# MingyuKim87/Safe_Denoiser

Measured on AMD Instinct MI355X. Metric: images/sec (512x512, 50 steps, SD-v1.4 + repellency), higher is better.
Workload: dtype bf16; 1 GPU; README-default end to end (safree = svf = lra = true, safree_neg_prompt_config.json:26-28): token ids -> CLIP -> SAFREE projection -> DDPM 50 steps x UNet on 3 guidance branches with per-prompt text switching + safe_denoiser.yaml repellency (kernel_fast, M=515, sigma 3.15, scale .33, margin 1.6, window 780<=t<=1000) -> VAE decode -> uint8 512x512 images; SD-v1.4 UNet / CLIP / VAE with random weigh; guidance_branches=3, text_encoder_precision=bf16x3, prompts_per_batch=64, latent_repeat=3, renoise_draws_rank0=3520, parallelism=prompt-shard x1

## Files before the change

safe_denoiser_amd/csrc/sdn_attn.hip:

```cpp
#include <stdlib.h>

#include <type_traits>

#include "sdn_common.h"
#include "sdn_ops.h"

namespace sdn_attn_detail {

typedef __attribute__((ext_vector_type(4))) short s16x4;
typedef __attribute__((ext_vector_type(16))) float f32x16;
typedef __attribute__((ext_vector_type(4))) unsigned int u32x4;

#if defined(__HIP_DEVICE_COMPILE__)
__device__ __forceinline__ __amdgpu_buffer_rsrc_t make_rsrc(const void* p, unsigned bytes) {
  return __builtin_amdgcn_make_buffer_rsrc(const_cast<void*>(p), 0, (int)bytes, 0x00020000);
}
typedef __attribute__((address_space(3))) void* lds_ptr_t;
#endif

#ifdef SDN_ATTN_STAMPS
#define SDN_ATS_DECL unsigned long long ats_prev = 0, ats_sum[7] = {0, 0, 0, 0, 0, 0, 0};
#define SDN_ATS_T0 unsigned long long ats_t0; asm volatile("s_memtime %0\n\ts_waitcnt lgkmcnt(0)" : "=s"(ats_t0)::"memory");
#define SDN_ATS_MARK(I)                                                                         \
  {                                                                                             \
    unsigned long long t_;                                                                      \
    asm volatile("s_memtime %0\n\ts_waitcnt lgkmcnt(0)" : "=s"(t_)::"memory");                  \
    if ((I) >= 0) ats_sum[(I) < 0 ? 0 : (I)] += t_ - ats_prev;                                  \
    ats_prev = t_;                                                                              \
  }
#define SDN_ATS_FLUSH                                                                           \
  if (g_attn_stamps && lane == 0)                                                               \
    for (int i_ = 0; i_ < 7; ++i_) g_attn_stamps[((long)blockIdx.x * 4 + wid) * 7 + i_] = ats_sum[i_];
__device__ unsigned long long* g_attn_stamps = nullptr;
#define SDN_ATS_PRO ats_sum[5] = ats_prev - ats_t0;
#else
#define SDN_ATS_DECL
#define SDN_ATS_T0
#define SDN_ATS_PRO
#define SDN_ATS_MARK(I)
#define SDN_ATS_FLUSH
#endif

constexpr int THREADS = 256;
[[maybe_unused]] constexpr int KV = 64;
constexpr int QB = 128;

struct AttnArgs {
  const unsigned short* q; const unsigned short* k; const unsigned short* v; unsigned short* out;
  int nq, nk, ldq, ldk, ldv, ldo;
  float c;
  int heads, nqb, npairs;
  const unsigned short* q2; const unsigned short* k2; const unsigned short* v2; unsigned short* out2;
  int n1, ldq2, ldk2, ldv2, ldo2;
  int head_inner;
  int causal; const int* kmask;
  int nomax;
  const float* bias;
};

template <bool SEG>
__device__ __forceinline__ const unsigned short* row_ptr(const unsigned short* p1, const unsigned short* p2, int ld1,
                                                          int ld2, int n1, int n, int b, int row) {
  if (SEG && row >= n1) return p2 + ((long)b * (n - n1) + (row - n1)) * ld2;
  return p1 + ((long)b * (SEG ? n1 : n) + row) * ld1;
}

template <typename T, int HD, bool SEG, bool MASK = false, bool DMA = !SEG, int QS = 1, bool BIAS = false>
__global__ void __launch_bounds__(THREADS)
k_attn(const AttnArgs a) {
#if defined(__HIP_DEVICE_COMPILE__)
  SDN_ATS_T0
  constexpr int KQ = (HD + 15) / 16;
  constexpr int NDB = (HD + 31) / 32;
  constexpr bool ONES = (HD % 32) != 0;
  static_assert(!BIAS || (MASK && DMA && QS == 1), "the biased form extends the masked single-buffer instance");
  constexpr bool OFFSET_FREE = T::kDtype == 0 && !BIAS;
  constexpr bool CENTRED = T::kDtype == 1 && !SEG && !MASK && DMA && (KQ * 16 > HD);
  constexpr bool CENTRED_SUB = T::kDtype == 1 && !MASK && !CENTRED;
  constexpr bool QSCALED = OFFSET_FREE || CENTRED || CENTRED_SUB;
  static_assert(!CENTRED || ((HD % 32) != 0 && HD - 16 * (KQ - 1) == 8), "centred form: row sums by the ones column, column HD = element 0 of the h = 1 lanes");
  constexpr int CH = HD / 8;
#ifndef SDN_ATTN_VCH40
#define SDN_ATTN_VCH40 5
#endif
  constexpr int KCH = HD == 40 ? 5 : CH + 1;
  constexpr int VCH = HD == 40 ? SDN_ATTN_VCH40 : (HD == 160 ? 20 : 12);
  constexpr int KSTR = DMA ? KCH * 16 : KQ * 32 + 16;
  constexpr int VSTR_PAD = (NDB * 16) % 64 == 16 || (NDB * 16) % 64 == 48 ? NDB * 64 : NDB * 64 + 64;
  constexpr int VSTR = DMA ? VCH * 16 : VSTR_PAD;
  constexpr int STAGE = KV * KSTR + KV * VSTR;
  constexpr int ZOFF = 2 * STAGE;
  constexpr int NLOAD = (2 * KV * CH + THREADS - 1) / THREADS;
  constexpr int BOFF = ZOFF + 64;
  __shared__ __attribute__((aligned(1024))) unsigned char smem[BIAS ? BOFF + 4096 : 2 * STAGE + 48];

  constexpr bool kLateDma = HD == 40;
#ifdef SDN_ATTN_NO_ASM_TR
  constexpr bool kAsmTrOn = false;
#else
  constexpr bool kAsmTrOn = true;
#endif
  const int tid = threadIdx.x, lane = tid & 63;
  const int wid = __builtin_amdgcn_readfirstlane(tid >> 6);
  const int r = lane & 31, h = lane >> 5;
  int pair, qblk;
  {
    const int nqb = a.nqb, npairs = a.npairs, id = blockIdx.x;
    if (a.head_inner) {
      const int x = id & 7, j = id >> 3;
      const int hh = j % a.heads, rest = j / a.heads;
      qblk = rest % nqb;
      pair = ((rest / nqb) * 8 + x) * a.heads + hh;
    } else if ((npairs & 7) == 0) {
      const int x = id & 7, j = id >> 3;
      pair = (j / nqb) * 8 + x; qblk = j - (j / nqb) * nqb;
    } else {
      pair = id / nqb; qblk = id - pair * nqb;
    }
  }
  const int head = pair % a.heads, b = pair / a.heads;
  const int q0 = qblk * (QB * QS) + wid * (32 * QS);
  bool qvalid[QS];
#pragma unroll
  for (int qs = 0; qs < QS; ++qs) qvalid[qs] = q0 + 32 * qs + r < a.nq;

  if (tid == 8) *reinterpret_cast<unsigned*>(smem + ZOFF + 32) = 0u;
  if constexpr (DMA) {
    if (tid < 8) *reinterpret_cast<unsigned*>(smem + ZOFF + tid * 4) = tid == 0 ? (T::pack2(1.0f, 0.0f) & 0xffffu) : 0u;
  } else {
    const unsigned one16 = T::pack2(1.0f, 0.0f) & 0xffffu;
    for (int e = tid; e < 2 * KV; e += THREADS) {
      unsigned char* sK = smem + (e / KV) * STAGE + (e % KV) * KSTR;
      unsigned char* sV = smem + (e / KV) * STAGE + KV * KSTR + (e % KV) * VSTR;
      for (int c = CH * 16; c < KQ * 32; c += 4) *reinterpret_cast<unsigned*>(sK + c) = 0u;
      for (int c = CH * 16; c < NDB * 64; c += 4) *reinterpret_cast<unsigned*>(sV + c) = (ONES && c == CH * 16) ? one16 : 0u;
    }
  }

  if constexpr (BIAS) {
    const int L = 2 * a.nk - 1;
    for (int e = tid; e < L; e += THREADS)
      reinterpret_cast<float*>(smem + BOFF)[e] = a.bias[(long)head * L + e] * 1.4426950408889634f;
  }

  typename T::v8 qf[QS][KQ];
#pragma unroll
  for (int qs = 0; qs < QS; ++qs)
#pragma unroll
  for (int s = 0; s < KQ; ++s) {
    const int dc = 16 * s + 8 * h;
    u32x4 v = (u32x4){0u, 0u, 0u, 0u};
    if (qvalid[qs] && dc < HD)
      v = *reinterpret_cast<const u32x4*>(row_ptr<SEG>(a.q, a.q2, a.ldq, a.ldq2, a.n1, a.nq, b, q0 + 32 * qs + r) + head * HD + dc);
    if (QSCALED) {
      v.x = T::pack2(T::to_f(v.x & 0xffff) * a.c, T::to_f(v.x >> 16) * a.c);
      v.y = T::pack2(T::to_f(v.y & 0xffff) * a.c, T::to_f(v.y >> 16) * a.c);
      v.z = T::pack2(T::to_f(v.z & 0xffff) * a.c, T::to_f(v.z >> 16) * a.c);
      v.w = T::pack2(T::to_f(v.w & 0xffff) * a.c, T::to_f(v.w >> 16) * a.c);
    }
    qf[qs][s] = *reinterpret_cast<typename T::v8*>(&v);
  }

  u32x4 stg[NLOAD];
  int ld_row[NLOAD], ld_dst[NLOAD];
  const unsigned short* ld_src[NLOAD];
  long ld_stride[NLOAD];
#pragma unroll
  for (int i = 0; i < NLOAD; ++i) {
    int e = tid + i * THREADS;
    const bool live = e < 2 * KV * CH;
    if (!live) e = 2 * KV * CH - 1;
    const int isv = e >= KV * CH;
    const int e2 = isv ? e - KV * CH : e;
    const int row = e2 / CH, ch = e2 - row * CH;
    ld_row[i] = row;
    ld_dst[i] = live ? (isv ? KV * KSTR + row * VSTR : row * KSTR) + ch * 16 : -1;
    ld_src[i] = (isv ? a.v + (long)b * a.nk * a.ldv : a.k + (long)b * a.nk * a.ldk) + head * HD + ch * 8;
    ld_stride[i] = isv ? a.ldv : a.ldk;
    if (SEG) { ld_stride[i] = isv; ld_src[i] = nullptr; ld_row[i] |= ch << 16; }
  }
  auto g_load = [&](int t) {
    const int k0 = t * KV;
#pragma unroll
    for (int i = 0; i < NLOAD; ++i) {
      if (SEG) {
        const int krow = min(k0 + (ld_row[i] & 0xffff), a.nk - 1), ch = ld_row[i] >> 16;
        const unsigned short* rp = ld_stride[i] ? row_ptr<true>(a.v, a.v2, a.ldv, a.ldv2, a.n1, a.nk, b, krow)
                                                : row_ptr<true>(a.k, a.k2, a.ldk, a.ldk2, a.n1, a.nk, b, krow);
        stg[i] = *reinterpret_cast<const u32x4*>(rp + head * HD + ch * 8);
      } else {
        const int krow = min(k0 + ld_row[i], a.nk - 1);
        stg[i] = *reinterpret_cast<const u32x4*>(ld_src[i] + (long)krow * ld_stride[i]);
      }
    }
  };
  auto s_store = [&](int buf, int t) {
    const int k0 = t * KV;
#pragma unroll
    for (int i = 0; i < NLOAD; ++i) {
      if (ld_dst[i] >= 0) {
        const u32x4 v = (k0 + (ld_row[i] & 0xffff) < a.nk) ? stg[i] : (u32x4){0u, 0u, 0u, 0u};
        *reinterpret_cast<u32x4*>(smem + buf * STAGE + ld_dst[i]) = v;
      }
    }
  };

  constexpr int NPIECE = (KCH + VCH + 3) / 4;
  unsigned dma_off[NPIECE];
  if constexpr (DMA) {
#pragma unroll
    for (int i = 0; i < NPIECE; ++i) {
      const int p = wid + 4 * i;
      const bool isv = p >= KCH;
      const int e = (isv ? p - KCH : p) * 64 + lane;
      const int rowc = isv ? VCH : KCH;
      const int row = e / rowc, ch = e - row * rowc;
      dma_off[i] = ch < CH ? (unsigned)(((long)row * (isv ? a.ldv : a.ldk) + head * HD + ch * 8) * 2) : 0x80000000u;
    }
  }
  auto dma_issue = [&](int buf, int t) {
    const long k0 = (long)t * KV;
    const unsigned short *kb_, *vb_;
    long rk, rv;
    if (SEG && k0 >= a.n1) {
      const long kk = k0 - a.n1, n2 = a.nk - a.n1;
      kb_ = a.k2 + ((long)b * n2 + kk) * a.ldk2; vb_ = a.v2 + ((long)b * n2 + kk) * a.ldv2;
      rk = ((n2 - kk - 1) * a.ldk2 + a.heads * HD) * 2; rv = ((n2 - kk - 1) * a.ldv2 + a.heads * HD) * 2;
    } else {
      const long n1 = SEG ? a.n1 : a.nk;
      kb_ = a.k + ((long)b * n1 + k0) * a.ldk; vb_ = a.v + ((long)b * n1 + k0) * a.ldv;
      rk = ((n1 - k0 - 1) * a.ldk + a.heads * HD) * 2; rv = ((n1 - k0 - 1) * a.ldv + a.heads * HD) * 2;
    }
    const __amdgpu_buffer_rsrc_t rs_k = make_rsrc(kb_, (unsigned)(rk > 0 ? rk : 0));
    const __amdgpu_buffer_rsrc_t rs_v = make_rsrc(vb_, (unsigned)(rv > 0 ? rv : 0));
#pragma unroll
    for (int i = 0; i < NPIECE; ++i) {
      const int p = wid + 4 * i;
      if (p < KCH)
        __builtin_amdgcn_raw_ptr_buffer_load_lds(rs_k, (lds_ptr_t)(smem + buf * STAGE + p * 1024), 16, dma_off[i], 0, 0, 0);
      else if (p < KCH + VCH)
        __builtin_amdgcn_raw_ptr_buffer_load_lds(rs_v, (lds_ptr_t)(smem + buf * STAGE + KV * KSTR + (p - KCH) * 1024), 16,
                                                 dma_off[i], 0, 0, 0);
    }
  };

  SDN_ATS_DECL
  f32x16 o[QS][NDB];
  float l_tot[QS];
  auto run_pass = [&](auto safe_c) __attribute__((always_inline)) {
  constexpr bool safe = decltype(safe_c)::value;
  float m_run[QS], l_run[QS];
  float m_hi[QS];
#pragma unroll
  for (int qs = 0; qs < QS; ++qs) {
#pragma unroll
    for (int d = 0; d < NDB; ++d)
#pragma unroll
      for (int i = 0; i < 16; ++i) o[qs][d][i] = 0.f;
    m_run[qs] = OFFSET_FREE ? 0.f : -1e30f; l_run[qs] = 0.f; m_hi[qs] = -1e30f;
    if constexpr (CENTRED) {
      u32x4 v = *reinterpret_cast<u32x4*>(&qf[qs][KQ - 1]);
      if (h == 1) v.x &= 0xffff0000u;
      qf[qs][KQ - 1] = *reinterpret_cast<typename T::v8*>(&v);
    }
  }

  const int gi = lane & 15, gq = gi >> 2, gp = gi & 3, gcol = 16 * ((lane >> 4) & 1);

  const int ntiles = (a.nk + KV - 1) / KV;
  if constexpr (DMA) {
    dma_issue(0, 0);
    asm volatile("s_waitcnt vmcnt(0)" ::: "memory");
  } else {
    g_load(0);
    s_store(0, 0);
  }
  __syncthreads();

  SDN_ATS_MARK(-1)
  SDN_ATS_PRO
  for (int t = 0; t < ntiles; ++t) {
    const int buf = t & 1;
    const unsigned char* sK = smem + buf * STAGE;
    const unsigned char* sV = sK + KV * KSTR;
    if (t + 1 < ntiles) {
      if constexpr (DMA) { if (!kLateDma) dma_issue(buf ^ 1, t + 1); }
      else g_load(t + 1);
    }

    f32x16 st[QS][2];
    constexpr bool kPreloadK = QS == 2;
    typename T::v8 kfa[kPreloadK ? 2 : 1][kPreloadK ? KQ : 1];
    if constexpr (kPreloadK) {
#pragma unroll
      for (int kb = 0; kb < 2; ++kb)
#pragma unroll
        for (int s = 0; s < KQ; ++s) {
          const unsigned char* kp = sK + (32 * kb + r) * KSTR + (16 * s + 8 * h) * 2;
          if (DMA && 16 * s + 16 > HD) { if (16 * s + 8 * h >= HD) kp = smem + ZOFF + (CENTRED ? 0 : 16); }
          kfa[kb][s] = *reinterpret_cast<const typename T::v8*>(kp);
        }
      __builtin_amdgcn_sched_barrier(0);
    }
    __builtin_amdgcn_s_setprio(1);
#pragma unroll
    for (int kb = 0; kb < 2; ++kb) {
#pragma unroll
      for (int qs = 0; qs < QS; ++qs)
#pragma unroll
        for (int i = 0; i < 16; ++i) st[qs][kb][i] = 0.f;
#pragma unroll
      for (int s = 0; s < KQ; ++s) {
        typename T::v8 kf;
        if constexpr (kPreloadK) {
          kf = kfa[kb][s];
        } else {
          const unsigned char* kp = sK + (32 * kb + r) * KSTR + (16 * s + 8 * h) * 2;
          if (DMA && 16 * s + 16 > HD) { if (16 * s + 8 * h >= HD) kp = smem + ZOFF + (CENTRED ? 0 : 16); }
          kf = *reinterpret_cast<const typename T::v8*>(kp);
        }
#pragma unroll
        for (int qs = 0; qs < QS; ++qs) st[qs][kb] = T::mfma32(kf, qf[qs][s], st[qs][kb]);
      }
    }
    __builtin_amdgcn_s_setprio(0);
    if constexpr (DMA && kLateDma) { if (t + 1 < ntiles) dma_issue(buf ^ 1, t + 1); }
    if constexpr (BIAS) {
      const float* sb = reinterpret_cast<const float*>(smem + BOFF);
      const int k0 = t * KV, last = 2 * a.nk - 2;
#pragma unroll
      for (int kb = 0; kb < 2; ++kb)
#pragma unroll
        for (int i = 0; i < 16; ++i) {
          const int key = k0 + 32 * kb + (i & 3) + 8 * (i >> 2) + 4 * h;
#pragma unroll
          for (int qs = 0; qs < QS; ++qs) {
            const int idx = key - (q0 + 32 * qs + r) + a.nk - 1;
            st[qs][kb][i] = fmaf(st[qs][kb][i], a.c, sb[min(max(idx, 0), last)]);
          }
        }
    }
    if constexpr (MASK) {
      const int k0 = t * KV;
#pragma unroll
      for (int kb = 0; kb < 2; ++kb)
#pragma unroll
        for (int i = 0; i < 16; ++i) {
          const int key = k0 + 32 * kb + (i & 3) + 8 * (i >> 2) + 4 * h;
#pragma unroll
          for (int qs = 0; qs < QS; ++qs) {
            bool off = key >= a.nk || (a.causal && key > q0 + 32 * qs + r);
            if (!off && a.kmask) off = a.kmask[(long)b * a.nk + key] == 0;
            if (off) st[qs][kb][i] = -1e30f;
          }
        }
    } else if ((t + 1) * KV > a.nk) {
      const int k0 = t * KV;
#pragma unroll
      for (int kb = 0; kb < 2; ++kb)
#pragma unroll
// ... 216 lines not shown
    } else {
      l_tot[qs] = l_run[qs] + __shfl_xor(l_run[qs], 32, 64);
    }
    if constexpr (CENTRED || CENTRED_SUB) bad |= !(l_tot[qs] >= 0x1p-10f && l_tot[qs] <= 0x1p15f);
    else bad |= !(l_tot[qs] >= 0x1p-64f && l_tot[qs] <= 0x1p64f);
  }
  return bad;
  };
  bool rerun = true;
  if constexpr (OFFSET_FREE || CENTRED || CENTRED_SUB) {
    if (a.nomax) {
      const bool bad = run_pass(std::false_type{});
      if (__builtin_amdgcn_ballot_w64(bad) != 0 && lane == 0) *reinterpret_cast<volatile unsigned*>(smem + ZOFF + 32) = 1u;
      __syncthreads();
      rerun = *reinterpret_cast<volatile unsigned*>(smem + ZOFF + 32) != 0u;
    }
  }
  if (rerun) run_pass(std::true_type{});
#pragma unroll
  for (int qs = 0; qs < QS; ++qs) {
  const float inv = 1.f / l_tot[qs];
  if (qvalid[qs]) {
    unsigned short* orow = const_cast<unsigned short*>(row_ptr<SEG>(a.out, a.out2, a.ldo, a.ldo2, a.n1, a.nq, b, q0 + 32 * qs + r)) + head * HD;
#pragma unroll
    for (int d = 0; d < NDB; ++d)
#pragma unroll
      for (int tq = 0; tq < 4; ++tq) {
        const int dc = 32 * d + 8 * tq + 4 * h;
        if (dc < HD) {
          uint2 pk;
          pk.x = T::pack2(o[qs][d][4 * tq + 0] * inv, o[qs][d][4 * tq + 1] * inv);
          pk.y = T::pack2(o[qs][d][4 * tq + 2] * inv, o[qs][d][4 * tq + 3] * inv);
          *reinterpret_cast<uint2*>(orow + dc) = pk;
        }
      }
  }
  }
  SDN_ATS_MARK(6)
  SDN_ATS_FLUSH
#endif
}

struct AttnPArgs {
  const unsigned short* q; const unsigned short* k; const unsigned short* v;
  void* out;
  int nq, nk, ldq, ldk, ldv, ldo, lo_q, lo_kv;
  float c;
  int heads, nqb, npairs, triple;
};

template <int HD, int QS, int NW, int KVT>
__global__ void __launch_bounds__(64 * NW)
k_attn_x3p(const AttnPArgs a) {
#if defined(__HIP_DEVICE_COMPILE__)
  typedef SdnBF16 T;
  constexpr int KQ = (HD + 15) / 16, NDB = (HD + 31) / 32, CH = HD / 8;
  constexpr bool ONES = HD % 32 != 0;
  constexpr int KCH = HD == 40 ? 5 : CH + 1, VCH = HD == 40 ? 5 : (HD == 160 ? 20 : 12);
  constexpr int KSTR = KCH * 16, VSTR = VCH * 16, NKB = KVT / 32;
  constexpr int KP = (KVT * KCH + 63) / 64, VP = (KVT * VCH + 63) / 64;
  constexpr int OFF_KL = KP * 1024, OFF_VH = 2 * KP * 1024, OFF_VL = OFF_VH + VP * 1024;
  constexpr int STAGE = 2 * (KP + VP) * 1024;
  constexpr int ZOFF = 2 * STAGE;
  constexpr int NP = 2 * (KP + VP), NPIECE = (NP + NW - 1) / NW;
  __shared__ __attribute__((aligned(1024))) unsigned char smem[2 * STAGE + 32];
  const int tid = threadIdx.x, lane = tid & 63;
  const int wid = __builtin_amdgcn_readfirstlane(tid >> 6);
  const int r = lane & 31, h = lane >> 5;
  int pair, qblk;
  {
    const int nqb = a.nqb, id = blockIdx.x;
    if ((a.npairs & 7) == 0) { const int x = id & 7, j = id >> 3; pair = (j / nqb) * 8 + x; qblk = j - (j / nqb) * nqb; }
    else { pair = id / nqb; qblk = id - pair * nqb; }
  }
  const int head = pair % a.heads, b = pair / a.heads;
  const int q0 = qblk * (32 * NW * QS) + wid * (32 * QS);
  bool qvalid[QS];
#pragma unroll
  for (int qs = 0; qs < QS; ++qs) qvalid[qs] = q0 + 32 * qs + r < a.nq;
  if (tid < 8) *reinterpret_cast<unsigned*>(smem + ZOFF + tid * 4) = tid == 0 ? (T::pack2(1.0f, 0.0f) & 0xffffu) : 0u;

  typename T::v8 qh[QS][KQ], ql[QS][KQ];
#pragma unroll
  for (int qs = 0; qs < QS; ++qs)
#pragma unroll
    for (int s = 0; s < KQ; ++s) {
      const int dc = 16 * s + 8 * h;
      u32x4 vh = (u32x4){0u, 0u, 0u, 0u}, vl = vh;
      if (qvalid[qs] && dc < HD) {
        const unsigned short* qp = a.q + ((long)b * a.nq + q0 + 32 * qs + r) * a.ldq + head * HD + dc;
        vh = *reinterpret_cast<const u32x4*>(qp); vl = *reinterpret_cast<const u32x4*>(qp + a.lo_q);
      }
      qh[qs][s] = *reinterpret_cast<typename T::v8*>(&vh); ql[qs][s] = *reinterpret_cast<typename T::v8*>(&vl);
    }

  unsigned dma_off[NPIECE];
#pragma unroll
  for (int i = 0; i < NPIECE; ++i) {
    const int p = wid + NW * i;
    const bool isv = p >= 2 * KP;
    const int pi = isv ? (p - 2 * KP) % VP : p % KP;
    const int e = pi * 64 + lane;
    const int rowc = isv ? VCH : KCH;
    const int row = e / rowc, ch = e - row * rowc;
    dma_off[i] = (ch < CH && row < KVT) ? (unsigned)(((long)row * (isv ? a.ldv : a.ldk) + head * HD + ch * 8) * 2) : 0x80000000u;
  }
  auto dma_issue = [&](int buf, int t) {
    const long k0 = (long)t * KVT;
    const unsigned short* kb_ = a.k + ((long)b * a.nk + k0) * a.ldk;
    const unsigned short* vb_ = a.v + ((long)b * a.nk + k0) * a.ldv;
    const long rk = ((a.nk - k0 - 1) * a.ldk + a.heads * HD) * 2, rv = ((a.nk - k0 - 1) * a.ldv + a.heads * HD) * 2;
    const __amdgpu_buffer_rsrc_t rs_kh = make_rsrc(kb_, (unsigned)(rk > 0 ? rk : 0));
    const __amdgpu_buffer_rsrc_t rs_kl = make_rsrc(kb_ + a.lo_kv, (unsigned)(rk > 0 ? rk : 0));
    const __amdgpu_buffer_rsrc_t rs_vh = make_rsrc(vb_, (unsigned)(rv > 0 ? rv : 0));
    const __amdgpu_buffer_rsrc_t rs_vl = make_rsrc(vb_ + a.lo_kv, (unsigned)(rv > 0 ? rv : 0));
    unsigned char* st = smem + buf * STAGE;
#pragma unroll
    for (int i = 0; i < NPIECE; ++i) {
      const int p = wid + NW * i;
      if (p < KP) __builtin_amdgcn_raw_ptr_buffer_load_lds(rs_kh, (lds_ptr_t)(st + p * 1024), 16, dma_off[i], 0, 0, 0);
      else if (p < 2 * KP) __builtin_amdgcn_raw_ptr_buffer_load_lds(rs_kl, (lds_ptr_t)(st + OFF_KL + (p - KP) * 1024), 16, dma_off[i], 0, 0, 0);
      else if (p < 2 * KP + VP) __builtin_amdgcn_raw_ptr_buffer_load_lds(rs_vh, (lds_ptr_t)(st + OFF_VH + (p - 2 * KP) * 1024), 16, dma_off[i], 0, 0, 0);
      else if (p < NP) __builtin_amdgcn_raw_ptr_buffer_load_lds(rs_vl, (lds_ptr_t)(st + OFF_VL + (p - 2 * KP - VP) * 1024), 16, dma_off[i], 0, 0, 0);
    }
  };

  f32x16 o[QS][NDB];
  float m_run[QS];
  [[maybe_unused]] float l_run[QS];
#pragma unroll
  for (int qs = 0; qs < QS; ++qs) {
#pragma unroll
    for (int d = 0; d < NDB; ++d)
#pragma unroll
      for (int i = 0; i < 16; ++i) o[qs][d][i] = 0.f;
    m_run[qs] = -1e30f; l_run[qs] = 0.f;
  }
  const int gi = lane & 15, gq = gi >> 2, gp = gi & 3, gcol = 16 * ((lane >> 4) & 1);
  const int ntiles = (a.nk + KVT - 1) / KVT;
  dma_issue(0, 0);
  asm volatile("s_waitcnt vmcnt(0)" ::: "memory");
  __syncthreads();
  for (int t = 0; t < ntiles; ++t) {
    const int buf = t & 1;
    const unsigned char* sKh = smem + buf * STAGE;
    const unsigned char* sVh = sKh + OFF_VH;
    f32x16 st[QS][NKB];
    __builtin_amdgcn_s_setprio(1);
#pragma unroll
    for (int kb = 0; kb < NKB; ++kb) {
#pragma unroll
      for (int qs = 0; qs < QS; ++qs)
#pragma unroll
        for (int i = 0; i < 16; ++i) st[qs][kb][i] = 0.f;
#pragma unroll
      for (int s = 0; s < KQ; ++s) {
        const unsigned char* kp = sKh + (32 * kb + r) * KSTR + (16 * s + 8 * h) * 2;
        const unsigned char* kq = kp + OFF_KL;
        if (16 * s + 16 > HD) { if (16 * s + 8 * h >= HD) kp = kq = smem + ZOFF + 16; }
        const typename T::v8 kfh = *reinterpret_cast<const typename T::v8*>(kp), kfl = *reinterpret_cast<const typename T::v8*>(kq);
#pragma unroll
        for (int qs = 0; qs < QS; ++qs) st[qs][kb] = T::mfma32(kfl, qh[qs][s], st[qs][kb]);
#pragma unroll
        for (int qs = 0; qs < QS; ++qs) st[qs][kb] = T::mfma32(kfh, ql[qs][s], st[qs][kb]);
#pragma unroll
        for (int qs = 0; qs < QS; ++qs) st[qs][kb] = T::mfma32(kfh, qh[qs][s], st[qs][kb]);
      }
    }
    __builtin_amdgcn_s_setprio(0);
    if (t + 1 < ntiles) dma_issue(buf ^ 1, t + 1);
    if ((t + 1) * KVT > a.nk) {
      const int k0 = t * KVT;
#pragma unroll
      for (int kb = 0; kb < NKB; ++kb)
#pragma unroll
        for (int i = 0; i < 16; ++i) {
          const int key = k0 + 32 * kb + (i & 3) + 8 * (i >> 2) + 4 * h;
          if (key >= a.nk) {
#pragma unroll
            for (int qs = 0; qs < QS; ++qs) st[qs][kb][i] = -1e30f;
          }
        }
    }
#pragma unroll
    for (int qs = 0; qs < QS; ++qs) {
      float mx = st[qs][0][0];
#pragma unroll
      for (int kb = 0; kb < NKB; ++kb)
#pragma unroll
        for (int i = 0; i < 16; ++i) mx = fmaxf(mx, st[qs][kb][i]);
      {
        const unsigned u = __float_as_uint(mx);
        const auto sw = __builtin_amdgcn_permlane32_swap(u, u, false, false);
        mx = fmaxf(__uint_as_float(sw[0]), __uint_as_float(sw[1]));
      }
      const float m_new = fmaxf(m_run[qs], mx);
      const float mc = m_new * a.c;
      if (__builtin_amdgcn_ballot_w64(m_new != m_run[qs]) != 0) {
        const float alpha = __builtin_amdgcn_exp2f((m_run[qs] - m_new) * a.c);
        if (!ONES) l_run[qs] *= alpha;
#pragma unroll
        for (int d = 0; d < NDB; ++d)
#pragma unroll
          for (int i = 0; i < 16; ++i) o[qs][d][i] *= alpha;
        m_run[qs] = m_new;
      }
#pragma unroll
      for (int kb = 0; kb < NKB; ++kb)
#pragma unroll
        for (int i = 0; i < 16; ++i) st[qs][kb][i] = __builtin_amdgcn_exp2f(fmaf(st[qs][kb][i], a.c, -mc));
      if (!ONES) {
        float ps = 0.f;
#pragma unroll
        for (int kb = 0; kb < NKB; ++kb)
#pragma unroll
          for (int i = 0; i < 16; ++i) ps += st[qs][kb][i];
        l_run[qs] += ps;
      }
    }
    __builtin_amdgcn_s_setprio(1);
#pragma unroll
    for (int kb = 0; kb < NKB; ++kb)
#pragma unroll
      for (int s2 = 0; s2 < 2; ++s2) {
        typename T::v8 ph[QS], pl[QS];
#pragma unroll
        for (int qs = 0; qs < QS; ++qs) {
          u32x4 wh, wl;
          const float* pv = reinterpret_cast<const float*>(&st[qs][kb]) + 8 * s2;
          unsigned hh[4], ll[4];
#pragma unroll
          for (int e = 0; e < 4; ++e) {
            hh[e] = T::pack2(pv[2 * e], pv[2 * e + 1]);
            ll[e] = T::pack2(pv[2 * e] - T::to_f(hh[e] & 0xffff), pv[2 * e + 1] - T::to_f(hh[e] >> 16));
          }
          wh.x = hh[0]; wh.y = hh[1]; wh.z = hh[2]; wh.w = hh[3];
          wl.x = ll[0]; wl.y = ll[1]; wl.z = ll[2]; wl.w = ll[3];
          ph[qs] = *reinterpret_cast<typename T::v8*>(&wh); pl[qs] = *reinterpret_cast<typename T::v8*>(&wl);
        }
        const int keyb = 32 * kb + 16 * s2 + 4 * h + gq;
#pragma unroll
        for (int d = 0; d < NDB; ++d) {
          const unsigned char* pa = sVh + keyb * VSTR + (32 * d + gcol + 4 * gp) * 2;
          const unsigned char* pb = pa + 8 * VSTR;
          const unsigned char* la = pa + (OFF_VL - OFF_VH);
          const unsigned char* lb = pb + (OFF_VL - OFF_VH);
          if (32 * d + 32 > HD) {
            const int col = 32 * d + gcol + 4 * gp;
            if (col >= HD) { pa = pb = smem + ZOFF + ((ONES && col == HD) ? 0 : 8); la = lb = smem + ZOFF + 8; }
          }
          union { s16x4 hlf[2]; typename T::v8 full; } vfh, vfl;
          vfh.hlf[0] = __builtin_amdgcn_ds_read_tr16_b64_v4i16((__attribute__((address_space(3))) s16x4*)(pa));
          vfh.hlf[1] = __builtin_amdgcn_ds_read_tr16_b64_v4i16((__attribute__((address_space(3))) s16x4*)(pb));
          vfl.hlf[0] = __builtin_amdgcn_ds_read_tr16_b64_v4i16((__attribute__((address_space(3))) s16x4*)(la));
          vfl.hlf[1] = __builtin_amdgcn_ds_read_tr16_b64_v4i16((__attribute__((address_space(3))) s16x4*)(lb));
#pragma unroll
          for (int qs = 0; qs < QS; ++qs) o[qs][d] = T::mfma32(vfl.full, ph[qs], o[qs][d]);
#pragma unroll
          for (int qs = 0; qs < QS; ++qs) o[qs][d] = T::mfma32(vfh.full, pl[qs], o[qs][d]);
#pragma unroll
          for (int qs = 0; qs < QS; ++qs) o[qs][d] = T::mfma32(vfh.full, ph[qs], o[qs][d]);
        }
      }
    __builtin_amdgcn_s_setprio(0);
    asm volatile("s_waitcnt vmcnt(0)" ::: "memory");
    __syncthreads();
  }
#pragma unroll
  for (int qs = 0; qs < QS; ++qs) {
    float l_tot;
    if constexpr (ONES) {
      constexpr int row = HD % 32, ri = (row >> 3) * 4 + (row & 3);
      static_assert(((row >> 2) & 1) == 0, "ones row must live in lane half 0");
      l_tot = __shfl(o[qs][NDB - 1][ri], r, 64);
    } else {
      l_tot = l_run[qs] + __shfl_xor(l_run[qs], 32, 64);
    }
    const float inv = 1.f / l_tot;
    if (!qvalid[qs]) continue;
    const long qrow = (long)b * a.nq + q0 + 32 * qs + r;
#pragma unroll
    for (int d = 0; d < NDB; ++d)
#pragma unroll
      for (int tq = 0; tq < 4; ++tq) {
        const int dc = 32 * d + 8 * tq + 4 * h;
        if (dc < HD) {
          const float v0 = o[qs][d][4 * tq + 0] * inv, v1 = o[qs][d][4 * tq + 1] * inv, v2 = o[qs][d][4 * tq + 2] * inv, v3 = o[qs][d][4 * tq + 3] * inv;
          if (a.triple) {
            unsigned short* o3 = reinterpret_cast<unsigned short*>(a.out) + qrow * 3 * a.ldo + head * HD + dc;
            uint2 hi, lo;
            hi.x = T::pack2(v0, v1); hi.y = T::pack2(v2, v3);
            lo.x = T::pack2(v0 - T::to_f(hi.x & 0xffff), v1 - T::to_f(hi.x >> 16));
            lo.y = T::pack2(v2 - T::to_f(hi.y & 0xffff), v3 - T::to_f(hi.y >> 16));
            *reinterpret_cast<uint2*>(o3) = hi; *reinterpret_cast<uint2*>(o3 + a.ldo) = lo; *reinterpret_cast<uint2*>(o3 + 2 * a.ldo) = hi;
          } else {
            *reinterpret_cast<sdn_f32x4*>(reinterpret_cast<float*>(a.out) + qrow * a.ldo + head * HD + dc) = (sdn_f32x4){v0, v1, v2, v3};
          }
        }
      }
  }
#endif
}

static int g_attn_qs2 = 1;
static int g_attn_nomax = 1;

template <typename T, int HD>
int launch(const AttnArgs& a, int batch, int heads, hipStream_t st) {
  if (a.bias) {
    if constexpr (HD == 64) {
      if (a.q2 || a.causal) return SDN_E_INVALID;
      hipLaunchKernelGGL((k_attn<T, HD, false, true, true, 1, true>), dim3(a.nqb * a.npairs), dim3(THREADS), 0, st, a);
      return sdn_launch_status();
    } else {
      return SDN_E_INVALID;
    }
  }
  if (a.causal || a.kmask) {
    if constexpr (HD == 64) {
      if (a.q2) return SDN_E_INVALID;
      hipLaunchKernelGGL((k_attn<T, HD, false, true>), dim3(a.nqb * a.npairs), dim3(THREADS), 0, st, a);
      return sdn_launch_status();
    } else {
      return SDN_E_INVALID;
    }
  }
  if (a.q2) {
    if constexpr (HD == 64) {
      if (a.n1 % KV == 0 && a.ldk == a.ldk2 && a.ldv == a.ldv2) {
        hipLaunchKernelGGL((k_attn<T, HD, true, false, true>), dim3(a.nqb * a.npairs), dim3(THREADS), 0, st, a);
        return sdn_launch_status();
      }
    }
    hipLaunchKernelGGL((k_attn<T, HD, true>), dim3(a.nqb * a.npairs), dim3(THREADS), 0, st, a);
  } else {
    if constexpr (HD == 40) {
      if (a.nk > 2 * KV && a.nq >= 2 * QB && g_attn_qs2) {
        AttnArgs a2 = a;
        a2.nqb = (a.nq + 2 * QB - 1) / (2 * QB);
        hipLaunchKernelGGL((k_attn<T, HD, false, false, true, 2>), dim3(a2.nqb * a2.npairs), dim3(THREADS), 0, st, a2);
        return sdn_launch_status();
      }
    }
    hipLaunchKernelGGL((k_attn<T, HD, false>), dim3(a.nqb * a.npairs), dim3(THREADS), 0, st, a);
  }
  return sdn_launch_status();
}

static int g_attn_head_inner = 1;

template <typename T>
int run(const void* q, const void* k, const void* v, void* out, int32_t batch, int32_t heads, int32_t nq, int32_t nk,
        int32_t head_dim, int32_t ldq, int32_t ldk, int32_t ldv, int32_t ldo, float scale, void* stream,
        const sdn_attn_segment2* s2 = nullptr, int causal = 0, const int* kmask = nullptr, const float* bias = nullptr) {
  if (!q || !k || !v || !out || batch < 0 || heads <= 0 || nq <= 0 || nk <= 0) return SDN_E_INVALID;
  if ((ldq & 7) || (ldk & 7) || (ldv & 7) || (ldo & 3) || nk > 65535) return SDN_E_INVALID;
  if (ldq < heads * head_dim || ldk < heads * head_dim || ldv < heads * head_dim || ldo < heads * head_dim)
    return SDN_E_INVALID;
  auto al = [](const void* p, int n) { return (reinterpret_cast<uintptr_t>(p) & (n - 1)) == 0; };
  if (!al(q, 16) || !al(k, 16) || !al(v, 16) || !al(out, 8)) return SDN_E_INVALID;
  if (batch == 0) return SDN_OK;
  AttnArgs a{(const unsigned short*)q, (const unsigned short*)k, (const unsigned short*)v, (unsigned short*)out,
             nq, nk, ldq, ldk, ldv, ldo, scale * 1.4426950408889634f, heads, (nq + QB - 1) / QB, batch * heads,
             nullptr, nullptr, nullptr, nullptr, 0, 0, 0, 0, 0, 0, causal, kmask, g_attn_nomax, bias};
  if (!s2 && nk <= 2 * KV && (batch & 7) == 0 && g_attn_head_inner) a.head_inner = 1;
  if (causal && nq != nk) return SDN_E_INVALID;
  if (s2) {
    if (!s2->q2 || !s2->k2 || !s2->v2 || !s2->out2 || s2->n1 <= 0 || s2->n1 >= nq || nq != nk) return SDN_E_INVALID;
    if ((s2->ldq2 & 7) || (s2->ldk2 & 7) || (s2->ldv2 & 7) || (s2->ldo2 & 3)) return SDN_E_INVALID;
    if (!al(s2->q2, 16) || !al(s2->k2, 16) || !al(s2->v2, 16) || !al(s2->out2, 8)) return SDN_E_INVALID;
    a.q2 = (const unsigned short*)s2->q2; a.k2 = (const unsigned short*)s2->k2; a.v2 = (const unsigned short*)s2->v2;
    a.out2 = (unsigned short*)s2->out2; a.n1 = s2->n1;
    a.ldq2 = s2->ldq2; a.ldk2 = s2->ldk2; a.ldv2 = s2->ldv2; a.ldo2 = s2->ldo2;
  }
  hipStream_t st = (hipStream_t)stream;
  switch (head_dim) {
    case 40: return launch<T, 40>(a, batch, heads, st);
    case 64: return launch<T, 64>(a, batch, heads, st);
    case 80: return launch<T, 80>(a, batch, heads, st);
    case 160: return launch<T, 160>(a, batch, heads, st);
    default: return SDN_E_INVALID;
  }
}

}

#ifdef SDN_ATTN_STAMPS
extern "C" int sdn_debug_set_attn_stamps(void* p) {
  return (int)hipMemcpyToSymbol(HIP_SYMBOL(sdn_attn_detail::g_attn_stamps), &p, sizeof(p));
}
#endif
extern "C" void sdn_debug_set_attn_qs2(int on) { sdn_attn_detail::g_attn_qs2 = on; }
extern "C" void sdn_debug_set_attn_nomax(int on) { sdn_attn_detail::g_attn_nomax = on; }
extern "C" int sdn_attention_bf16(const void* q, const void* k, const void* v, void* out, int32_t batch,
                                  int32_t heads, int32_t nq, int32_t nk, int32_t head_dim, int32_t ldq,
                                  int32_t ldk, int32_t ldv, int32_t ldo, float scale, void* stream) {
  return sdn_attn_detail::run<SdnBF16>(q, k, v, out, batch, heads, nq, nk, head_dim, ldq, ldk, ldv, ldo, scale, stream);
}
extern "C" int sdn_attention_f16(const void* q, const void* k, const void* v, void* out, int32_t batch,
                                 int32_t heads, int32_t nq, int32_t nk, int32_t head_dim, int32_t ldq,
                                 int32_t ldk, int32_t ldv, int32_t ldo, float scale, void* stream) {
  return sdn_attn_detail::run<SdnF16>(q, k, v, out, batch, heads, nq, nk, head_dim, ldq, ldk, ldv, ldo, scale, stream);
}
extern "C" int sdn_joint_attention(int32_t dtype, const void* q, const void* k, const void* v, void* out,
                                   const sdn_attn_segment2* seg2, int32_t batch, int32_t heads, int32_t n_total,
                                   int32_t head_dim, int32_t ldq, int32_t ldk, int32_t ldv, int32_t ldo, float scale,
                                   void* stream) {
  if (!seg2) return SDN_E_INVALID;
  if (dtype == 1)
    return sdn_attn_detail::run<SdnF16>(q, k, v, out, batch, heads, n_total, n_total, head_dim, ldq, ldk, ldv, ldo, scale,
                                        stream, seg2);
  return sdn_attn_detail::run<SdnBF16>(q, k, v, out, batch, heads, n_total, n_total, head_dim, ldq, ldk, ldv, ldo, scale,
                                       stream, seg2);
}

extern "C" int sdn_masked_attention(int32_t dtype, const void* q, const void* k, const void* v, void* out,
                                    const int32_t* key_mask, int32_t causal, int32_t batch, int32_t heads, int32_t n,
                                    int32_t head_dim, int32_t ldq, int32_t ldk, int32_t ldv, int32_t ldo, float scale,
                                    void* stream) {
  if (!causal && !key_mask) return SDN_E_INVALID;
  if (dtype == 1)
    return sdn_attn_detail::run<SdnF16>(q, k, v, out, batch, heads, n, n, head_dim, ldq, ldk, ldv, ldo, scale, stream, nullptr,
                                        causal ? 1 : 0, key_mask);
  return sdn_attn_detail::run<SdnBF16>(q, k, v, out, batch, heads, n, n, head_dim, ldq, ldk, ldv, ldo, scale, stream, nullptr,
                                       causal ? 1 : 0, key_mask);
}

extern "C" int sdn_bias_attention(int32_t dtype, const void* q, const void* k, const void* v, void* out, const float* bias,
                                  const int32_t* key_mask, int32_t batch, int32_t heads, int32_t n, int32_t head_dim, int32_t ldq,
                                  int32_t ldk, int32_t ldv, int32_t ldo, float scale, void* stream) {
  if (!bias || (reinterpret_cast<uintptr_t>(bias) & 3) || n < 2 || n > 512 || head_dim != 64 || dtype < 0 || dtype > 1) return SDN_E_INVALID;
  if (dtype == 1)
    return sdn_attn_detail::run<SdnF16>(q, k, v, out, batch, heads, n, n, head_dim, ldq, ldk, ldv, ldo, scale, stream, nullptr, 0,
                                        key_mask, bias);
  return sdn_attn_detail::run<SdnBF16>(q, k, v, out, batch, heads, n, n, head_dim, ldq, ldk, ldv, ldo, scale, stream, nullptr, 0,
                                       key_mask, bias);
}

extern "C" void sdn_debug_set_attn_head_inner(int on) { sdn_attn_detail::g_attn_head_inner = on; }

extern "C" int sdn_attention_x3_pairs(const void* q, const void* k, const void* v, int32_t lo_offset_q, int32_t lo_offset_kv, void* out, int32_t batch,
                                      int32_t heads, int32_t nq, int32_t nk, int32_t head_dim, int32_t ldq, int32_t ldk, int32_t ldv,
                                      int32_t ldo, float scale, int32_t triple, void* stream) {
  using namespace sdn_attn_detail;
  if (!q || !k || !v || !out || batch < 0 || heads <= 0 || nq <= 0 || nk <= 0 || lo_offset_q <= 0 || lo_offset_kv <= 0) return SDN_E_INVALID;
  if ((ldq & 7) || (ldk & 7) || (ldv & 7) || (lo_offset_q & 7) || (lo_offset_kv & 7) || (ldo & 3) || nk > 65535) return SDN_E_INVALID;
  if (lo_offset_q < heads * head_dim || lo_offset_kv < heads * head_dim || ldq < lo_offset_q + heads * head_dim ||
      ldk < lo_offset_kv + heads * head_dim || ldv < lo_offset_kv + heads * head_dim || ldo < heads * head_dim)
    return SDN_E_INVALID;
  auto al = [](const void* p, int n) { return (reinterpret_cast<uintptr_t>(p) & (n - 1)) == 0; };
  if (!al(q, 16) || !al(k, 16) || !al(v, 16) || !al(out, 16)) return SDN_E_INVALID;
  if (head_dim != 40 && head_dim != 80 && head_dim != 160) return SDN_E_INVALID;
  if ((long)nk * ldk * 2 >= (1L << 31) || (long)nk * ldv * 2 >= (1L << 31)) return SDN_E_INVALID;
  if (batch == 0) return SDN_OK;
  static const int qs_env = getenv("SDN_X3P_QS") ? atoi(getenv("SDN_X3P_QS")) : 0;
  static const int nw_env = getenv("SDN_X3P_NW") ? atoi(getenv("SDN_X3P_NW")) : 0;
  int qs = (head_dim == 40 && nq >= 2 * QB) ? 2 : 1;
  int nw = (head_dim == 80 || head_dim == 160) && nq >= 2 * QB ? 8 : 4;
  if (head_dim == 40 && qs_env) qs = qs_env == 2 ? 2 : 1;
  if (nw_env) nw = nw_env == 8 ? 8 : 4;
  if (head_dim != 40) qs = 1;
  if (head_dim == 40 && qs == 2) nw = 4;
  const int qper = 32 * nw * qs;
  AttnPArgs a{(const unsigned short*)q, (const unsigned short*)k, (const unsigned short*)v, out, nq, nk, ldq, ldk, ldv, ldo, lo_offset_q, lo_offset_kv,
              scale * 1.4426950408889634f, heads, (nq + qper - 1) / qper, batch * heads, triple ? 1 : 0};
  const unsigned grid = (unsigned)(a.nqb * a.npairs);
  hipStream_t st = (hipStream_t)stream;
  if (head_dim == 40) {
    if (qs == 2) hipLaunchKernelGGL((k_attn_x3p<40, 2, 4, 64>), dim3(grid), dim3(256), 0, st, a);
    else if (nw == 8) hipLaunchKernelGGL((k_attn_x3p<40, 1, 8, 64>), dim3(grid), dim3(512), 0, st, a);
    else hipLaunchKernelGGL((k_attn_x3p<40, 1, 4, 64>), dim3(grid), dim3(256), 0, st, a);
  } else if (head_dim == 80) {
    if (nw == 8) hipLaunchKernelGGL((k_attn_x3p<80, 1, 8, 64>), dim3(grid), dim3(512), 0, st, a);
    else hipLaunchKernelGGL((k_attn_x3p<80, 1, 4, 64>), dim3(grid), dim3(256), 0, st, a);
  } else {
    if (nw == 8) hipLaunchKernelGGL((k_attn_x3p<160, 1, 8, 32>), dim3(grid), dim3(512), 0, st, a);
    else hipLaunchKernelGGL((k_attn_x3p<160, 1, 4, 32>), dim3(grid), dim3(256), 0, st, a);
  }
  return sdn_launch_status();
}
```

Measured before the change: 8.318 images/sec.

## Add short-key attention kernel with whole-KV LDS residency and q-block splitting

Adds a dedicated attention kernel for non-64 head dims when the key length is at most 96, which is the case for cross-attention over CLIP's 77 text tokens. It loads all of K and V into LDS once per block and does a single-pass softmax with no online rescaling, then loops over several query blocks so the K/V load is reused. The grid is sized to about 16 workgroups per CU, and the next query tile is prefetched while the current one is computed. The risks are numerics when exponents are large (bf16 uses a guard offset and no row max) and a heuristic grid split that assumes 256 CUs.

```diff
diff --git a/safe_denoiser_amd/csrc/sdn_attn.hip b/safe_denoiser_amd/csrc/sdn_attn.hip
--- a/safe_denoiser_amd/csrc/sdn_attn.hip
+++ b/safe_denoiser_amd/csrc/sdn_attn.hip
@@ -1,5 +1,6 @@
 #include <stdlib.h>
 
+#include <algorithm>
 #include <type_traits>
 
 #include "sdn_common.h"
@@ -56,6 +57,7 @@
   int causal; const int* kmask;
   int nomax;
   const float* bias;
+  int bpw, nsplit;
 };
 
 template <bool SEG>
@@ -878,6 +880,220 @@
 #endif
 }
 
+constexpr int kShortBlocks = 3;
+
+template <typename T, int HD, int NKB>
+__global__ void __launch_bounds__(THREADS)
+k_attn_short(const AttnArgs a) {
+#if defined(__HIP_DEVICE_COMPILE__)
+  constexpr int KQ = (HD + 15) / 16;
+  constexpr int NDB = (HD + 31) / 32;
+  constexpr bool ONES = (HD % 32) != 0;
+  constexpr int CH = HD / 8;
+  constexpr int KCH = HD == 40 ? 5 : CH + 1;
+  constexpr int VCH = HD == 40 ? 5 : (HD == 160 ? 20 : 12);
+  constexpr int KSTR = KCH * 16, VSTR = VCH * 16;
+  constexpr int NKP = 32 * NKB;
+  constexpr int VOFF = NKP * KSTR, ZOFF = VOFF + NKP * VSTR;
+  __shared__ __attribute__((aligned(16))) unsigned char smem[ZOFF + 32];
+
+  const int tid = threadIdx.x, lane = tid & 63;
+  const int wid = __builtin_amdgcn_readfirstlane(tid >> 6);
+  const int r = lane & 31, h = lane >> 5;
+  int pair, part;
+  {
+    const int ns = a.nsplit, id = blockIdx.x;
+    if (a.head_inner) {
+      const int x = id & 7, j = id >> 3;
+      const int hh = j % a.heads, rest = j / a.heads;
+      part = rest % ns;
+      pair = ((rest / ns) * 8 + x) * a.heads + hh;
+    } else {
+      pair = id / ns; part = id - pair * ns;
+    }
+  }
+  const int head = pair % a.heads, b = pair / a.heads;
+  const int blk0 = part * a.bpw, blk1 = min(blk0 + a.bpw, a.nqb);
+  const int nk = a.nk;
+
+  const unsigned short* qbase = a.q + (long)b * a.nq * a.ldq + head * HD;
+  u32x4 qn[KQ];
+  auto load_q = [&](int blk) {
+    const int row = min(blk * QB + wid * 32 + r, a.nq - 1);
+#pragma unroll
+    for (int s = 0; s < KQ; ++s) {
+      const int dc = 16 * s + 8 * h;
+      qn[s] = *reinterpret_cast<const u32x4*>(qbase + (long)row * a.ldq + (dc < HD ? dc : 0));
+    }
+  };
+  typename T::v8 qf[KQ];
+  auto scale_q = [&]() {
+#pragma unroll
+    for (int s = 0; s < KQ; ++s) {
+      u32x4 v = qn[s];
+      if (16 * s + 8 * h >= HD) v = (u32x4){0u, 0u, 0u, 0u};
+      v.x = T::pack2(T::to_f(v.x & 0xffff) * a.c, T::to_f(v.x >> 16) * a.c);
+      v.y = T::pack2(T::to_f(v.y & 0xffff) * a.c, T::to_f(v.y >> 16) * a.c);
+      v.z = T::pack2(T::to_f(v.z & 0xffff) * a.c, T::to_f(v.z >> 16) * a.c);
+      v.w = T::pack2(T::to_f(v.w & 0xffff) * a.c, T::to_f(v.w >> 16) * a.c);
+      qf[s] = *reinterpret_cast<typename T::v8*>(&v);
+    }
+  };
+  load_q(blk0);
+
+  {
+    const unsigned short* kb_ = a.k + (long)b * nk * a.ldk + head * HD;
+    const unsigned short* vb_ = a.v + (long)b * nk * a.ldv + head * HD;
+    for (int e = tid; e < NKP * CH; e += THREADS) {
+      const int row = e / CH, ch = e - row * CH;
+      const int src = min(row, nk - 1);
+      u32x4 kk = *reinterpret_cast<const u32x4*>(kb_ + (long)src * a.ldk + ch * 8);
+      u32x4 vv = *reinterpret_cast<const u32x4*>(vb_ + (long)src * a.ldv + ch * 8);
+      if (row >= nk) { kk = (u32x4){0u, 0u, 0u, 0u}; vv = kk; }
+      *reinterpret_cast<u32x4*>(smem + row * KSTR + ch * 16) = kk;
+      *reinterpret_cast<u32x4*>(smem + VOFF + row * VSTR + ch * 16) = vv;
+    }
+    if (tid < 8) *reinterpret_cast<unsigned*>(smem + ZOFF + tid * 4) = tid == 0 ? (T::pack2(1.0f, 0.0f) & 0xffffu) : 0u;
+  }
+  __syncthreads();
+
+  const unsigned char* sK = smem;
+  const unsigned char* sV = smem + VOFF;
+  const int gi = lane & 15, gq = gi >> 2, gp = gi & 3, gcol = 16 * ((lane >> 4) & 1);
+  scale_q();
+
+  f32x16 tail;
+  {
+#pragma unroll
+    for (int i = 0; i < 16; ++i) tail[i] = 32 * (NKB - 1) + (i & 3) + 8 * (i >> 2) + 4 * h >= nk ? -1e30f : 0.f;
+  }
+
+  for (int blk = blk0; blk < blk1; ++blk) {
+    const int q0 = blk * QB + wid * 32;
+    load_q(min(blk + 1, blk1 - 1));
+    f32x16 st[NKB];
+    __builtin_amdgcn_s_setprio(1);
+#pragma unroll
+    for (int kb = 0; kb < NKB; ++kb) {
+      if (kb == NKB - 1) {
+        st[kb] = tail;
+      } else {
+#pragma unroll
+        for (int i = 0; i < 16; ++i) st[kb][i] = 0.f;
+      }
+#pragma unroll
+      for (int s = 0; s < KQ; ++s) {
+        const unsigned char* kp = sK + (32 * kb + r) * KSTR + (16 * s + 8 * h) * 2;
+        if (16 * s + 16 > HD) { if (16 * s + 8 * h >= HD) kp = smem + ZOFF + 16; }
+        st[kb] = T::mfma32(*reinterpret_cast<const typename T::v8*>(kp), qf[s], st[kb]);
+      }
+    }
+    __builtin_amdgcn_s_setprio(0);
+
+    float mx = st[0][0];
+#pragma unroll
+    for (int kb = 0; kb < NKB; ++kb)
+#pragma unroll
+      for (int i = 0; i < 16; ++i) mx = fmaxf(mx, st[kb][i]);
+    {
+      const unsigned u = __float_as_uint(mx);
+      const auto sw = __builtin_amdgcn_permlane32_swap(u, u, false, false);
+      mx = fmaxf(__uint_as_float(sw[0]), __uint_as_float(sw[1]));
+    }
+    if constexpr (T::kDtype == 0) {
+      constexpr float kGuard = 64.f;
+      const float off = fabsf(mx) > kGuard ? mx : 0.f;
+      if (__builtin_amdgcn_ballot_w64(off != 0.f) != 0) {
+#pragma unroll
+        for (int kb = 0; kb < NKB; ++kb)
+#pragma unroll
+          for (int i = 0; i < 16; ++i) st[kb][i] = __builtin_amdgcn_exp2f(st[kb][i] - off);
+      } else {
+#pragma unroll
+        for (int kb = 0; kb < NKB; ++kb)
+#pragma unroll
+          for (int i = 0; i < 16; ++i) st[kb][i] = __builtin_amdgcn_exp2f(st[kb][i]);
+      }
+    } else {
+#pragma unroll
+      for (int kb = 0; kb < NKB; ++kb)
+#pragma unroll
+        for (int i = 0; i < 16; ++i) st[kb][i] = __builtin_amdgcn_exp2f(st[kb][i] - mx);
+    }
+    [[maybe_unused]] float l_run = 0.f;
+    if (!ONES) {
+#pragma unroll
+      for (int kb = 0; kb < NKB; ++kb)
+#pragma unroll
+        for (int i = 0; i < 16; ++i) l_run += st[kb][i];
+    }
+
+    f32x16 o[NDB];
+#pragma unroll
+    for (int d = 0; d < NDB; ++d)
+#pragma unroll
+      for (int i = 0; i < 16; ++i) o[d][i] = 0.f;
+    __builtin_amdgcn_s_setprio(1);
+#pragma unroll
+    for (int kb = 0; kb < NKB; ++kb)
+#pragma unroll
+      for (int s2 = 0; s2 < 2; ++s2) {
+        if (kb == NKB - 1 && s2 == 1) { if (32 * kb + 16 >= nk) continue; }
+        u32x4 pw;
+        pw.x = T::pack2(st[kb][8 * s2 + 0], st[kb][8 * s2 + 1]);
+        pw.y = T::pack2(st[kb][8 * s2 + 2], st[kb][8 * s2 + 3]);
+        pw.z = T::pack2(st[kb][8 * s2 + 4], st[kb][8 * s2 + 5]);
+        pw.w = T::pack2(st[kb][8 * s2 + 6], st[kb][8 * s2 + 7]);
+        const typename T::v8 pf = *reinterpret_cast<typename T::v8*>(&pw);
+        const int keyb = 32 * kb + 16 * s2 + 4 * h + gq;
+#pragma unroll
+        for (int d = 0; d < NDB; ++d) {
+          const unsigned char* pa = sV + keyb * VSTR + (32 * d + gcol + 4 * gp) * 2;
+          const unsigned char* pb = pa + 8 * VSTR;
+          if (32 * d + 32 > HD) {
+            const int col = 32 * d + gcol + 4 * gp;
+            if (col >= HD) pa = pb = smem + ZOFF + (ONES && col == HD ? 0 : 8);
+          }
+          union { s16x4 hlf[2]; typename T::v8 full; } vf;
+          vf.hlf[0] = __builtin_amdgcn_ds_read_tr16_b64_v4i16((__attribute__((address_space(3))) s16x4*)(pa));
+          vf.hlf[1] = __builtin_amdgcn_ds_read_tr16_b64_v4i16((__attribute__((address_space(3))) s16x4*)(pb));
+          o[d] = T::mfma32(vf.full, pf, o[d]);
+        }
+      }
+    __builtin_amdgcn_s_setprio(0);
+
+    float l_tot;
+    if (ONES) {
+      constexpr int row = HD % 32;
+      constexpr int ri = (row >> 3) * 4 + (row & 3);
+      static_assert(((row >> 2) & 1) == 0, "ones row must live in lane half 0");
+      l_tot = __shfl(o[NDB - 1][ri], r, 64);
+    } else {
+      l_tot = l_run + __shfl_xor(l_run, 32, 64);
+    }
+    const float inv = 1.f / l_tot;
+    scale_q();
+    __builtin_amdgcn_sched_barrier(0);
+    if (q0 + r < a.nq) {
+      unsigned short* orow = a.out + ((long)b * a.nq + q0 + r) * a.ldo + head * HD;
+#pragma unroll
+      for (int d = 0; d < NDB; ++d)
+#pragma unroll
+        for (int tq = 0; tq < 4; ++tq) {
+          const int dc = 32 * d + 8 * tq + 4 * h;
+          if (dc < HD) {
+            uint2 pk;
+            pk.x = T::pack2(o[d][4 * tq + 0] * inv, o[d][4 * tq + 1] * inv);
+            pk.y = T::pack2(o[d][4 * tq + 2] * inv, o[d][4 * tq + 3] * inv);
+            *reinterpret_cast<uint2*>(orow + dc) = pk;
+          }
+        }
+    }
+  }
+#endif
+}
+
+static int g_attn_short = 1;
 static int g_attn_qs2 = 1;
 static int g_attn_nomax = 1;
 
@@ -910,6 +1126,21 @@
     }
     hipLaunchKernelGGL((k_attn<T, HD, true>), dim3(a.nqb * a.npairs), dim3(THREADS), 0, st, a);
   } else {
+    if constexpr (HD != 64) {
+      if (a.nk <= 32 * kShortBlocks && g_attn_short) {
+        constexpr long kShortWgPerCu = 16, kCus = 256;
+        const long want = (g_attn_short > 1 ? g_attn_short : kShortWgPerCu) * kCus;
+        AttnArgs as = a;
+        const long bpw = std::min<long>(a.nqb, std::max<long>(1, (long)a.nqb * a.npairs / want));
+        as.nsplit = (int)((a.nqb + bpw - 1) / bpw);
+        as.bpw = (a.nqb + as.nsplit - 1) / as.nsplit;
+        const dim3 grid(as.nsplit * as.npairs);
+        if (a.nk > 64) hipLaunchKernelGGL((k_attn_short<T, HD, 3>), grid, dim3(THREADS), 0, st, as);
+        else if (a.nk > 32) hipLaunchKernelGGL((k_attn_short<T, HD, 2>), grid, dim3(THREADS), 0, st, as);
+        else hipLaunchKernelGGL((k_attn_short<T, HD, 1>), grid, dim3(THREADS), 0, st, as);
+        return sdn_launch_status();
+      }
+    }
     if constexpr (HD == 40) {
       if (a.nk > 2 * KV && a.nq >= 2 * QB && g_attn_qs2) {
         AttnArgs a2 = a;
@@ -968,6 +1199,7 @@
 #endif
 extern "C" void sdn_debug_set_attn_qs2(int on) { sdn_attn_detail::g_attn_qs2 = on; }
 extern "C" void sdn_debug_set_attn_nomax(int on) { sdn_attn_detail::g_attn_nomax = on; }
+extern "C" void sdn_debug_set_attn_short(int on) { sdn_attn_detail::g_attn_short = on; }
 extern "C" int sdn_attention_bf16(const void* q, const void* k, const void* v, void* out, int32_t batch,
                                   int32_t heads, int32_t nq, int32_t nk, int32_t head_dim, int32_t ldq,
                                   int32_t ldk, int32_t ldv, int32_t ldo, float scale, void* stream) {
```

Result: no change. 8.337 images/sec (median of 4 runs) (+0.2%).
